# yosungho/LineTR

Measured on AMD Instinct MI355X. Metric: line_descriptors_per_sec, higher is better.
Workload: dtype f32 in/out; GEMMs as 6 bf16-split MFMA products, fp32 accumulate (fp32-faithful); 1 GPU; cfg3: 64 pairs/GPU of 640x480, 200 lines/image -> 199 sub-lines x 21 tokens, d_model=256, seeded weights; pairs_per_gpu=64, collective=none

## Files before the change

### linetr_amd/csrc/lt_attn_fused.h

```cpp
#pragma once
#include "lt_st_image.h"
#include "lt_attn.h"

namespace lt {

constexpr int FQA_W_BYTES = 3 * 4 * ST_RB;
constexpr int FQA_SLOT = FQA_W_BYTES + 256 * 64;
constexpr int FQA_KEYS = 128;
constexpr int FQA_LDS = 4 * FQA_SLOT;

__global__ __launch_bounds__(512) void sig_qkv_attn_kernel(const float* __restrict__ z ,
                                                           const unsigned char* __restrict__ Wst ,
                                                           const float* __restrict__ bqkv ,
                                                           const int* __restrict__ cu_sub, float* __restrict__ out ) {
  extern __shared__ __attribute__((aligned(1024))) unsigned char fq_smem[];
  const int img = blockIdx.x, head = blockIdx.y;
  const int n0 = cu_sub[img], Ni = cu_sub[img + 1] - n0;
  if (Ni <= 0) return;
  const int tid = threadIdx.x, lane = tid & 63;
  const int wave = __builtin_amdgcn_readfirstlane(tid >> 6);
  const int h2 = lane >> 5, lq = lane & 31;
  const int q = wave * 32 + lq;
  const bool wave_active = wave * 32 < Ni;
  constexpr int RBW = 3 * D / 16, NK = D / 16;

  const int n_dma = wave < 2 ? 5 : 4;
  const unsigned lane16 = lane * 16;
  auto issue_one = [&](int d, int k, int slot) {
    const int x = wave + 8 * d;
    unsigned char* dst = fq_smem + slot * FQA_SLOT + x * 1024;
    if (x < 18) {
      const unsigned char* g = Wst + ((int64_t)k * RBW + (x / 6) * 16 + head * 4) * ST_RB + (x % 6) * 1024;
      LT_GLDS(g + lane16, dst, 0);
    } else {
      int row = (x - 18) * 16 + (lane >> 2);
      row = row < Ni ? row : Ni - 1;
      const float* g = z + (int64_t)(n0 + row) * D + k * 16 + (((lane & 3) - ((lane >> 4) & 3)) & 3) * 4;
      LT_GLDS(g, dst, 0);
    }
  };
  auto issue_step = [&](int k, int slot) {
#pragma unroll
    for (int d = 0; d < 5; ++d)
      if (d < n_dma) issue_one(d, k, slot);
  };
  auto wait_dma = [&](int steps) {
    if (steps <= 0) asm volatile("s_waitcnt vmcnt(0)" ::: "memory");
    else if (wave < 2) {
      if (steps == 1) asm volatile("s_waitcnt vmcnt(5)" ::: "memory");
      else asm volatile("s_waitcnt vmcnt(10)" ::: "memory");
    } else {
      if (steps == 1) asm volatile("s_waitcnt vmcnt(4)" ::: "memory");
      else asm volatile("s_waitcnt vmcnt(8)" ::: "memory");
    }
  };
#pragma unroll
  for (int k = 0; k < 4; ++k) issue_step(k, k);
  f32x16 acc[6];
  {
    const float* bp = bqkv + head * DH + 4 * h2;
#pragma unroll
    for (int i = 0; i < 6; ++i)
#pragma unroll
      for (int bq = 0; bq < 4; ++bq) {
        const f32x4 v = *reinterpret_cast<const f32x4*>(bp + (i >> 1) * D + (i & 1) * 32 + 8 * bq);
#pragma unroll
        for (int c = 0; c < 4; ++c) acc[i][4 * bq + c] = v[c];
      }
  }
  wait_dma(2);
  __builtin_amdgcn_s_barrier();
  asm volatile("" ::: "memory");

  const int lfrag = ((lane >> 4) & 1) * ST_RB + (lane >> 5) * 256 + (lane & 15) * 16;
  const int zrot = (lq >> 2) & 3;
  const int zoff0 = FQA_W_BYTES + (wave * 32 + lq) * 64 + ((2 * h2 + zrot) & 3) * 16;
  const int zoff1 = FQA_W_BYTES + (wave * 32 + lq) * 64 + ((2 * h2 + 1 + zrot) & 3) * 16;
  using Terms = split_terms<3>;
  auto read_w = [&](int k, int i, int p, bf16x8 (&wf)[3]) {
    wf[p] = *reinterpret_cast<const bf16x8*>(fq_smem + (k & 3) * FQA_SLOT + lfrag + ((i >> 1) * 4 + (i & 1) * 2) * ST_RB + p * ST_CHUNK);
  };
  auto split_z = [&](const f32x4& x0, const f32x4& x1, bf16x8 (&zf)[3]) {
    unsigned a[3], b[3], c[3], d[3];
    split_pair<3>(x0[0], x0[1], a); split_pair<3>(x0[2], x0[3], b);
    split_pair<3>(x1[0], x1[1], c); split_pair<3>(x1[2], x1[3], d);
#pragma unroll
    for (int p = 0; p < 3; ++p) {
      union { bf16x8 v; unsigned w[4]; } u;
      u.w[0] = a[p]; u.w[1] = b[p]; u.w[2] = c[p]; u.w[3] = d[p];
      zf[p] = u.v;
    }
  };
  bf16x8 zfA[3], zfB[3], wfA[3], wfB[3];
  {
    const f32x4 x0 = *reinterpret_cast<const f32x4*>(fq_smem + zoff0), x1 = *reinterpret_cast<const f32x4*>(fq_smem + zoff1);
    split_z(x0, x1, zfA);
#pragma unroll
    for (int p = 0; p < 3; ++p) read_w(0, 0, p, wfA);
  }
  auto step = [&](int s, bf16x8 (&zc)[3], bf16x8 (&zn)[3]) {
    f32x4 zr0, zr1;
    const bool more = s + 1 < NK;
#pragma unroll
    for (int m = 0; m < 36; ++m) {
      const int i = m / 6, t = m % 6;
      bf16x8 (&wc)[3] = (i & 1) ? wfB : wfA;
      bf16x8 (&wn)[3] = (i & 1) ? wfA : wfB;
      acc[i] = mfma_split<0>(wc[Terms::pa(t)], zc[Terms::pb(t)], acc[i]);
      if (t < 3) {
        if (i < 5) read_w(s, i + 1, t, wn);
        else read_w(s + 1, 0, t, wn);
      }
      if (m == 3) zr0 = *reinterpret_cast<const f32x4*>(fq_smem + ((s + 1) & 3) * FQA_SLOT + zoff0);
      if (m == 4) zr1 = *reinterpret_cast<const f32x4*>(fq_smem + ((s + 1) & 3) * FQA_SLOT + zoff1);
      if (m == 15) split_z(zr0, zr1, zn);
      if (m >= 18 && m < 23 && s >= 1 && s + 3 < NK) { if (m - 18 < n_dma) issue_one(m - 18, s + 3, (s + 3) & 3); }
      __builtin_amdgcn_sched_barrier(0);
    }
    asm volatile("s_waitcnt lgkmcnt(0)" ::: "memory");
    if (more) {
      wait_dma(s + 3 < NK ? 1 : 0);
      __builtin_amdgcn_s_barrier();
      asm volatile("" ::: "memory");
    }
    __builtin_amdgcn_sched_barrier(0);
  };
#pragma unroll 1
  for (int s = 0; s < NK; s += 2) {
    step(s, zfA, zfB);
    step(s + 1, zfB, zfA);
  }
  asm volatile("s_waitcnt vmcnt(0)" ::: "memory");

  auto pieces = [&](const f32x16& a, float scale, float (&v)[16]) {
#pragma unroll
    for (int r = 0; r < 16; ++r) v[r] = a[r] * scale;
#pragma unroll
    for (int c = 0; c < 4; ++c) { halves_swap(v[c], v[4 + c]); halves_swap(v[8 + c], v[12 + c]); }
  };
  auto split_run = [&](const float* x, bf16x8 (&o)[3]) {
    unsigned a[3], b[3], c[3], d[3];
    split_pair<3>(x[0], x[1], a); split_pair<3>(x[2], x[3], b);
    split_pair<3>(x[4], x[5], c); split_pair<3>(x[6], x[7], d);
#pragma unroll
    for (int p = 0; p < 3; ++p) {
      union { bf16x8 v; unsigned w[4]; } u;
      u.w[0] = a[p]; u.w[1] = b[p]; u.w[2] = c[p]; u.w[3] = d[p];
      o[p] = u.v;
    }
  };
  bf16x8 qf[4][3];
#pragma unroll
  for (int i = 0; i < 2; ++i) {
    float v[16];
    pieces(acc[i], LOG2E, v);
    split_run(v, qf[2 * i]);
    split_run(v + 8, qf[2 * i + 1]);
  }
  unsigned char* Ks = fq_smem;
  unsigned char* Vs = fq_smem + FQA_KEYS * ATS_RK;
  auto stage_kv = [&]() {
    const int r = (wave & 3) * 32 + lq;
#pragma unroll
    for (int i = 2; i < 6; ++i) {
      float v[16];
      pieces(acc[i], 1.f, v);
      unsigned char* dst = (i < 4 ? Ks + r * ATS_RK : Vs + r * ATS_RV) + ((i & 1) * 32 + 8 * h2) * 2;
#pragma unroll
      for (int g = 0; g < 2; ++g) {
        bf16x8 pl[3];
        split_run(v + 8 * g, pl);
#pragma unroll
        for (int p = 0; p < 3; ++p) *reinterpret_cast<bf16x8*>(dst + p * 128 + g * 32) = pl[p];
      }
    }
  };
  f32x16 o0, o1;
#pragma unroll
  for (int r = 0; r < 16; ++r) { o0[r] = 0.f; o1[r] = 0.f; }
  float m = -INFINITY, l = 0.f;
  const unsigned v_base = (unsigned)(size_t)(Vs + (((lane & 15) >> 2) + 4 * h2) * ATS_RV + (((lane >> 4) & 1) * 16 + (lane & 3) * 4) * 2);
  auto chunk = [&](int kv0, auto kv_local) {
    constexpr int KL = decltype(kv_local)::value;
    constexpr int KB = KL >= 64 ? 64 : 0;
    const unsigned vb = v_base + KB * ATS_RV;
    u32x2 vrA[3][2], vrB[3][2];
    v_frags_tr<KL - KB, 0, false>(vb, vrA);
    f32x16 st;
#pragma unroll
    for (int r = 0; r < 16; ++r) st[r] = 0.f;
    const unsigned char* kp = Ks + (KL + lq) * ATS_RK + h2 * 16;
    bf16x8 kaA[3], kaB[3];
#pragma unroll
    for (int p = 0; p < 3; ++p) kaA[p] = *reinterpret_cast<const bf16x8*>(kp + p * 128);
#pragma unroll
    for (int m = 0; m < 24; ++m) {
      const int sq = m / 6, t = m % 6;
      bf16x8 (&kc)[3] = (sq & 1) ? kaB : kaA;
      bf16x8 (&kn)[3] = (sq & 1) ? kaA : kaB;
      st = mfma_split<0>(kc[split_terms<3>::pa(t)], qf[sq][split_terms<3>::pb(t)], st);
      if (t < 3 && sq < 3) kn[t] = *reinterpret_cast<const bf16x8*>(kp + t * 128 + (sq + 1) * 32);
      __builtin_amdgcn_sched_barrier(0);
    }
    if (kv0 + 32 > Ni) {
#pragma unroll
      for (int r = 0; r < 16; ++r)
        if (kv0 + (r & 3) + 8 * (r >> 2) + 4 * h2 >= Ni) st[r] = -INFINITY;
    }
    float mx = st[0];
#pragma unroll
    for (int r = 1; r < 16; ++r) mx = fmaxf(mx, st[r]);
    mx = xor32_max(mx);
    const float m_new = fmaxf(m, mx);
    float ps = 0.f;
#pragma unroll
    for (int r = 0; r < 16; ++r) { st[r] = __builtin_amdgcn_exp2f(st[r] - m_new); ps += st[r]; }
    ps = xor32_sum(ps);
    if (__any(m_new != m)) {
      const float alpha = __builtin_amdgcn_exp2f(m - m_new);
      l *= alpha;
#pragma unroll
      for (int r = 0; r < 16; ++r) { o0[r] *= alpha; o1[r] *= alpha; }
    }
    l += ps;
    m = m_new;
    bf16x8 pp0[3], pp1[3];
    {
      float sv[8];
#pragma unroll
      for (int e = 0; e < 8; ++e) sv[e] = st[e];
      split_run(sv, pp0);
    }
    auto pv = [&](u32x2 (&vr)[3][2], const bf16x8 (&pp)[3], f32x16& o) {
      bf16x8 va[3];
#pragma unroll
      for (int p = 0; p < 3; ++p) {
        union { bf16x8 v; unsigned u[4]; } x;
        x.u[0] = vr[p][0][0]; x.u[1] = vr[p][0][1]; x.u[2] = vr[p][1][0]; x.u[3] = vr[p][1][1];
        va[p] = x.v;
      }
      mma6(va, pp, o);
    };
    tr_wait(vrA);
    v_frags_tr<KL - KB, 1, false>(vb, vrB);
    pv(vrA, pp0, o0);
    __builtin_amdgcn_sched_barrier(0);
    {
      float sv[8];
#pragma unroll
      for (int e = 0; e < 8; ++e) sv[e] = st[8 + e];
      split_run(sv, pp1);
    }
    tr_wait(vrB);
    v_frags_tr<KL - KB + 16, 0, false>(vb, vrA);
    pv(vrB, pp0, o1);
    __builtin_amdgcn_sched_barrier(0);
    tr_wait(vrA);
    v_frags_tr<KL - KB + 16, 1, false>(vb, vrB);
    pv(vrA, pp1, o0);
    __builtin_amdgcn_sched_barrier(0);
    tr_wait(vrB);
    pv(vrB, pp1, o1);
  };
#pragma unroll
  for (int half = 0; half < 2; ++half) {
    if (half * FQA_KEYS >= Ni) break;
    __syncthreads();
    if ((wave >> 2) == half && wave_active) stage_kv();
    __syncthreads();
    if (!wave_active) continue;
    const int k0 = half * FQA_KEYS;
    if (k0 < Ni) chunk(k0, std::integral_constant<int, 0>{});
    if (k0 + 32 < Ni) chunk(k0 + 32, std::integral_constant<int, 32>{});
    if (k0 + 64 < Ni) chunk(k0 + 64, std::integral_constant<int, 64>{});
    if (k0 + 96 < Ni) chunk(k0 + 96, std::integral_constant<int, 96>{});
  }

  if (wave_active) {
    const float inv = 1.f / l;
    float* op = out + (int64_t)(n0 + (q < Ni ? q : Ni - 1)) * D + head * DH + 8 * h2;
#pragma unroll
    for (int dt = 0; dt < 2; ++dt) {
      float v[16];
      pieces(dt == 0 ? o0 : o1, inv, v);
      if (q < Ni) {
        *reinterpret_cast<f32x4*>(op + dt * 32) = f32x4{v[0], v[1], v[2], v[3]};
        *reinterpret_cast<f32x4*>(op + dt * 32 + 4) = f32x4{v[4], v[5], v[6], v[7]};
        *reinterpret_cast<f32x4*>(op + dt * 32 + 16) = f32x4{v[8], v[9], v[10], v[11]};
        *reinterpret_cast<f32x4*>(op + dt * 32 + 20) = f32x4{v[12], v[13], v[14], v[15]};
      }
    }
  }
}

}
```

Before: 10.56 million line-descriptors/s.

## Trim DMA to live rows, early-exit idle waves, skip empty PV half-tile

The per-wave DMA count now follows the real number of rows (Ni), so z rows beyond the image are no longer loaded, and the vmcnt waits are generalised to match. Inactive waves leave the compute path early and run only the barrier-matching DMA loop before returning. The final 16-key PV half-step is skipped when the chunk runs past Ni. These remove wasted loads and MFMA work on partial tiles, at the cost of a more complex barrier protocol that must stay matched across waves, and wave-uniform branching.

After: 10.61 million line-descriptors/s, median of 3. About the same (+0.4%).

```diff
diff --git a/linetr_amd/csrc/lt_attn_fused.h b/linetr_amd/csrc/lt_attn_fused.h
--- a/linetr_amd/csrc/lt_attn_fused.h
+++ b/linetr_amd/csrc/lt_attn_fused.h
@@ -24,7 +24,9 @@
   const bool wave_active = wave * 32 < Ni;
   constexpr int RBW = 3 * D / 16, NK = D / 16;
 
-  const int n_dma = wave < 2 ? 5 : 4;
+  const int n_x = 18 + 2 * ((Ni + 31) >> 5);
+  const int n_dma = (n_x - wave + 7) >> 3;
+  __builtin_assume(n_dma >= 2 && n_dma <= 5);
   const unsigned lane16 = lane * 16;
   auto issue_one = [&](int d, int k, int slot) {
     const int x = wave + 8 * d;
@@ -45,17 +47,39 @@
       if (d < n_dma) issue_one(d, k, slot);
   };
   auto wait_dma = [&](int steps) {
-    if (steps <= 0) asm volatile("s_waitcnt vmcnt(0)" ::: "memory");
-    else if (wave < 2) {
-      if (steps == 1) asm volatile("s_waitcnt vmcnt(5)" ::: "memory");
-      else asm volatile("s_waitcnt vmcnt(10)" ::: "memory");
-    } else {
-      if (steps == 1) asm volatile("s_waitcnt vmcnt(4)" ::: "memory");
-      else asm volatile("s_waitcnt vmcnt(8)" ::: "memory");
+    switch (steps <= 0 ? 0 : steps * n_dma) {
+      case 2: asm volatile("s_waitcnt vmcnt(2)" ::: "memory"); break;
+      case 3: asm volatile("s_waitcnt vmcnt(3)" ::: "memory"); break;
+      case 4: asm volatile("s_waitcnt vmcnt(4)" ::: "memory"); break;
+      case 5: asm volatile("s_waitcnt vmcnt(5)" ::: "memory"); break;
+      case 6: asm volatile("s_waitcnt vmcnt(6)" ::: "memory"); break;
+      case 8: asm volatile("s_waitcnt vmcnt(8)" ::: "memory"); break;
+      case 10: asm volatile("s_waitcnt vmcnt(10)" ::: "memory"); break;
+      default: asm volatile("s_waitcnt vmcnt(0)" ::: "memory"); break;
     }
   };
 #pragma unroll
   for (int k = 0; k < 4; ++k) issue_step(k, k);
+  if (!wave_active) {
+    wait_dma(2);
+    __builtin_amdgcn_s_barrier();
+#pragma unroll 1
+    for (int s = 0; s < NK; ++s) {
+      if (s >= 1 && s + 3 < NK) issue_step(s + 3, (s + 3) & 3);
+      asm volatile("s_waitcnt lgkmcnt(0)" ::: "memory");
+      if (s + 1 < NK) {
+        wait_dma(s + 3 < NK ? 1 : 0);
+        __builtin_amdgcn_s_barrier();
+      }
+    }
+    asm volatile("s_waitcnt vmcnt(0)" ::: "memory");
+    for (int half = 0; half < 2; ++half) {
+      if (half * FQA_KEYS >= Ni) break;
+      __syncthreads();
+      __syncthreads();
+    }
+    return;
+  }
   f32x16 acc[6];
   {
     const float* bp = bqkv + head * DH + 4 * h2;
@@ -224,7 +248,7 @@
     }
     l += ps;
     m = m_new;
-    bf16x8 pp0[3], pp1[3];
+    bf16x8 pp0[3];
     {
       float sv[8];
 #pragma unroll
@@ -242,33 +266,42 @@
       mma6(va, pp, o);
     };
     tr_wait(vrA);
-    v_frags_tr<KL - KB, 1, false>(vb, vrB);
-    pv(vrA, pp0, o0);
-    __builtin_amdgcn_sched_barrier(0);
-    {
-      float sv[8];
-#pragma unroll
-      for (int e = 0; e < 8; ++e) sv[e] = st[8 + e];
-      split_run(sv, pp1);
-    }
-    tr_wait(vrB);
-    v_frags_tr<KL - KB + 16, 0, false>(vb, vrA);
-    pv(vrB, pp0, o1);
-    __builtin_amdgcn_sched_barrier(0);
-    tr_wait(vrA);
-    v_frags_tr<KL - KB + 16, 1, false>(vb, vrB);
-    pv(vrA, pp1, o0);
-    __builtin_amdgcn_sched_barrier(0);
-    tr_wait(vrB);
-    pv(vrB, pp1, o1);
+    auto pv_steps = [&](auto second_step) {
+      v_frags_tr<KL - KB, 1, false>(vb, vrB);
+      pv(vrA, pp0, o0);
+      __builtin_amdgcn_sched_barrier(0);
+      if constexpr (!decltype(second_step)::value) {
+        tr_wait(vrB);
+        pv(vrB, pp0, o1);
+      } else {
+        bf16x8 pp1[3];
+        {
+          float sv[8];
+#pragma unroll
+          for (int e = 0; e < 8; ++e) sv[e] = st[8 + e];
+          split_run(sv, pp1);
+        }
+        tr_wait(vrB);
+        v_frags_tr<KL - KB + 16, 0, false>(vb, vrA);
+        pv(vrB, pp0, o1);
+        __builtin_amdgcn_sched_barrier(0);
+        tr_wait(vrA);
+        v_frags_tr<KL - KB + 16, 1, false>(vb, vrB);
+        pv(vrA, pp1, o0);
+        __builtin_amdgcn_sched_barrier(0);
+        tr_wait(vrB);
+        pv(vrB, pp1, o1);
+      }
+    };
+    if (kv0 + 16 >= Ni) pv_steps(std::false_type{});
+    else pv_steps(std::true_type{});
   };
 #pragma unroll
   for (int half = 0; half < 2; ++half) {
     if (half * FQA_KEYS >= Ni) break;
     __syncthreads();
-    if ((wave >> 2) == half && wave_active) stage_kv();
+    if ((wave >> 2) == half) stage_kv();
     __syncthreads();
-    if (!wave_active) continue;
     const int k0 = half * FQA_KEYS;
     if (k0 < Ni) chunk(k0, std::integral_constant<int, 0>{});
     if (k0 + 32 < Ni) chunk(k0 + 32, std::integral_constant<int, 32>{});
@@ -276,19 +309,17 @@
     if (k0 + 96 < Ni) chunk(k0 + 96, std::integral_constant<int, 96>{});
   }
 
-  if (wave_active) {
-    const float inv = 1.f / l;
-    float* op = out + (int64_t)(n0 + (q < Ni ? q : Ni - 1)) * D + head * DH + 8 * h2;
-#pragma unroll
-    for (int dt = 0; dt < 2; ++dt) {
-      float v[16];
-      pieces(dt == 0 ? o0 : o1, inv, v);
-      if (q < Ni) {
-        *reinterpret_cast<f32x4*>(op + dt * 32) = f32x4{v[0], v[1], v[2], v[3]};
-        *reinterpret_cast<f32x4*>(op + dt * 32 + 4) = f32x4{v[4], v[5], v[6], v[7]};
-        *reinterpret_cast<f32x4*>(op + dt * 32 + 16) = f32x4{v[8], v[9], v[10], v[11]};
-        *reinterpret_cast<f32x4*>(op + dt * 32 + 20) = f32x4{v[12], v[13], v[14], v[15]};
-      }
+  const float inv = 1.f / l;
+  float* op = out + (int64_t)(n0 + (q < Ni ? q : Ni - 1)) * D + head * DH + 8 * h2;
+#pragma unroll
+  for (int dt = 0; dt < 2; ++dt) {
+    float v[16];
+    pieces(dt == 0 ? o0 : o1, inv, v);
+    if (q < Ni) {
+      *reinterpret_cast<f32x4*>(op + dt * 32) = f32x4{v[0], v[1], v[2], v[3]};
+      *reinterpret_cast<f32x4*>(op + dt * 32 + 4) = f32x4{v[4], v[5], v[6], v[7]};
+      *reinterpret_cast<f32x4*>(op + dt * 32 + 16) = f32x4{v[8], v[9], v[10], v[11]};
+      *reinterpret_cast<f32x4*>(op + dt * 32 + 20) = f32x4{v[12], v[13], v[14], v[15]};
     }
   }
 }
```
